# mitsuba-renderer/mitsuba2

Hardware: AMD Instinct MI355X
Metric: Msamples/sec (whole node), 1080p/512spp path integrator (higher is better)
Workload: dtype f32

## Files before the change

### mitsuba2_amd/csrc/device/resident_kernel.h

```cpp
#ifndef MIW_KERNEL
#define MIW_KERNEL __global__
#endif
MIW_KERNEL __launch_bounds__(MIW_BLOCK) void k_init_pixels(RenderParams P, U4 *st_out, uint32_t *pixel_out, InitArgs A) {
    uint32_t lane = blockIdx.x * blockDim.x + threadIdx.x;
    if (lane >= P.n_lanes) return;
    uint32_t tile = lane >> A.bs2_log2, i = lane & ((1u << A.bs2_log2) - 1u);
    uint32_t b = A.tile_list ? A.tile_list[tile] : tile;
    uint32_t bx = b % A.blocks_x, by = b / A.blocks_x;
    uint32_t x, y;
    morton_decode2(i, x, y);
    int32_t bw = P.film.crop_w - (int32_t) (bx * A.bs), bh = P.film.crop_h - (int32_t) (by * A.bs);
    if (bw > (int32_t) A.bs) bw = (int32_t) A.bs;
    if (bh > (int32_t) A.bs) bh = (int32_t) A.bs;
    if ((int32_t) x >= bw || (int32_t) y >= bh) {
        U4 st; st.x = st.y = 0; st.z = LF_DONE; st.w = 0;
        st_out[lane] = st; pixel_out[lane] = 0;
        return;
    }
    uint32_t px = (uint32_t) P.film.crop_x + bx * A.bs + x, py = (uint32_t) P.film.crop_y + by * A.bs + y;
    pixel_out[lane] = px | (py << 16);
    st_out[lane] = lane_seed_state(A.base_seed + (uint64_t) A.block_ids[b] * (uint64_t) (A.bs * A.bs) + i);
}

struct TileArgs {
    const uint32_t *tile_list; uint32_t blocks_x, bs, bs2_log2;
    uint32_t side;
    uint32_t geom16;
};

#ifndef MIW_PLACE_PIECES
#define MIW_PLACE_PIECES 4
#endif
template <bool Placed = true, bool Clock = false, bool Groups = false, bool Jobs = true>
struct QueueWork {
    const LaneQueues *Q; uint32_t *next_pixel; uint32_t n_lanes, spp, lane, warn_negative;
    const FilmRec *film; const float *thr;
    uint32_t nq, per, q, dry, t_fetch;
    __device__ __forceinline__ void init_queues(uint32_t queues) {
        nq = Placed ? queues : 1u; per = nq > 1u ? MIW_PLACE_PIECES * 64u : n_lanes; q = 0u; dry = 0; t_fetch = 0;
        ticks = 0; quarter = 0; tail_prio = 0; sample_end_ = spp;
        if (Jobs) job_pend() = 0u;
        if (Placed && Q->simd_ids) {
            const uint32_t hw = (uint32_t) __builtin_amdgcn_s_getreg(4 | (0 << 6) | (31 << 11)),
                           xcc = (uint32_t) __builtin_amdgcn_s_getreg(20 | (0 << 6) | (3 << 11));
            const uint32_t key = ((xcc & 15u) << 10) | (((hw >> 13) & 7u) << 7) | (((hw >> 12) & 1u) << 6) | (((hw >> 8) & 15u) << 2) | ((hw >> 4) & 3u);
            if (nq > 1u) { const uint32_t id = Q->simd_ids[1u + key]; q = id < nq ? id : key % nq; }
            else if ((threadIdx.x & 63u) == 0u) Q->simd_ids[1u + key] = 1u;
        }
    }
    uint32_t ticks, quarter, tail_prio, sample_end_; uint32_t *prog;
    __device__ __forceinline__ void tick(uint32_t sample_idx, bool has_pixel) {
        if (!tail_prio) { ++ticks; return; }
        if ((uint32_t) __builtin_amdgcn_readfirstlane((int) ++ticks) & 15u) return;
        if (has_pixel) atomicMin(prog, sample_idx);
        const uint32_t v = *prog;
        *prog = 0xffffffffu;
        const uint32_t v4 = 4u * v, se = sample_end_;
        uint32_t qtr = v == 0xffffffffu ? 3u : (v4 >= se ? 1u : 0u) + (v4 >= 2u * se ? 1u : 0u) + (v4 >= 3u * se ? 1u : 0u);
        qtr = (uint32_t) __builtin_amdgcn_readfirstlane((int) qtr);
        if (qtr == quarter) return;
        quarter = qtr;
        if (qtr == 0u) __builtin_amdgcn_s_setprio(3); else if (qtr == 1u) __builtin_amdgcn_s_setprio(2);
        else if (qtr == 2u) __builtin_amdgcn_s_setprio(1); else __builtin_amdgcn_s_setprio(0);
    }
    __device__ __forceinline__ void enable_tail_prio(uint32_t sample_end, uint32_t *wave_word) {
        tail_prio = 1u; sample_end_ = sample_end; quarter = 0; prog = wave_word; *prog = 0xffffffffu; __builtin_amdgcn_s_setprio(3);
    }
    typedef uint32_t U4v __attribute__((ext_vector_type(4)));
    __device__ __forceinline__ static uint32_t &job_pend() { __shared__ uint32_t s_job_pend[MIW_BLOCK]; return s_job_pend[threadIdx.x & (MIW_BLOCK - 1)]; }
    __device__ __forceinline__ bool exhausted() const { return !Jobs || !Q->job_chunk || job_pend() == 0xffffffffu; }
    __device__ __forceinline__ uint32_t job_end(uint32_t sample_idx, uint32_t sample_end) const {
        const uint32_t r = spp - sample_idx;
        return Jobs && (r & (r - 1u)) == 0u && r >= Q->job_min ? sample_idx : sample_end;
    }
    __device__ __forceinline__ bool fetch_job(uint32_t &pixel, U4 &st) {
        for (;;) {
            const uint32_t parked = job_pend();
            if (parked == 0xffffffffu) return false;
            uint32_t id = parked - 1u;
            const bool fresh = parked == 0u;
            const unsigned long long b = __ballot(fresh);
            if (fresh) {
                const uint32_t me = threadIdx.x & 63u, leader = (uint32_t) __ffsll((long long) b) - 1u;
                uint32_t base = 0;
                if (me == leader) base = atomicAdd(next_pixel, (uint32_t) __popcll(b));
                base = (uint32_t) __shfl((int) base, (int) leader, 64);
                id = base + __builtin_amdgcn_mbcnt_hi((uint32_t) (b >> 32), __builtin_amdgcn_mbcnt_lo((uint32_t) b, 0u));
                if (id >= Q->job_total) { job_pend() = 0xffffffffu; return false; }
            }
            const uint32_t j = id / n_lanes, slot = id - j * n_lanes;
            const uint32_t px = Q->pixel[slot];
            U4v w;
#if defined(__HIP_DEVICE_COMPILE__)
            asm volatile("global_load_dwordx4 %0, %1, off sc1\n\ts_waitcnt vmcnt(0)" : "=&v"(w) : "v"(Q->st + slot) : "memory");
#endif
            if (w.z & LF_DONE) { job_pend() = 0u; continue; }
            if (w.w != (j ? spp - (Q->job_pow >> (j - 1u)) : 0u)) { job_pend() = id + 1u; return false; }
            job_pend() = 0u;
            lane = slot; pixel = px;
            st.x = w.x; st.y = w.y; st.z = w.z; st.w = w.w;
            return true;
        }
    }
    __device__ __forceinline__ bool fetch(uint32_t &pixel, U4 &st) {
        if (Jobs && Q->job_chunk) return fetch_job(pixel, st);
        for (;;) {
            if (!Placed) {
                const unsigned long long b = __ballot(1);
                const uint32_t me = threadIdx.x & 63u, leader = (uint32_t) __ffsll((long long) b) - 1u;
                uint32_t base = 0;
                if (me == leader) base = atomicAdd(next_pixel, (uint32_t) __popcll(b));
                base = (uint32_t) __shfl((int) base, (int) leader, 64);
                const uint32_t l = base + __builtin_amdgcn_mbcnt_hi((uint32_t) (b >> 32), __builtin_amdgcn_mbcnt_lo((uint32_t) b, 0u));
                if (l >= n_lanes) return false;
                lane = l;
                st = Q->st[lane];
                if (st.z & LF_DONE) continue;
                pixel = Q->pixel[lane];
                return true;
            }
            if (dry >= nq) {
                if (nq > 1u) Q->simd_ids[0] = 1u;
                return false;
            }
            if (nq > 1u && __hip_atomic_load(Q->simd_ids, __ATOMIC_RELAXED, __HIP_MEMORY_SCOPE_AGENT)) { dry = nq; return false; }
            const unsigned long long all = __ballot(1);
            const uint32_t me = threadIdx.x & 63u, leader = (uint32_t) __ffsll((long long) all) - 1u;
            const uint32_t q_lead = (uint32_t) __shfl((int) q, (int) leader, 64);
// ... 3 lines not shown
            uint32_t base = 0;
            if (me == leader) base = atomicAdd(next_pixel + q, (uint32_t) __popcll(b));
            base = (uint32_t) __shfl((int) base, (int) leader, 64);
            const uint32_t idx = base + __builtin_amdgcn_mbcnt_hi((uint32_t) (b >> 32), __builtin_amdgcn_mbcnt_lo((uint32_t) b, 0u));
            uint32_t l = idx;
            if (nq > 1u) {
                const uint32_t piece = idx < per ? Q->piece_list[q * MIW_PLACE_PIECES + (idx >> 6)] : 0xffffffffu;
                if (piece == 0xffffffffu) { q = q + 1u == nq ? 0u : q + 1u; ++dry; continue; }
                l = Q->lane_sorted[piece * Q->piece_a + (idx & 63u) * Q->piece_b];
                if (l >= n_lanes) continue;
            } else if (l >= n_lanes) { ++dry; continue; }
            lane = l;
            st = Q->st[lane];
            if (st.z & LF_DONE) continue;
            pixel = Q->pixel[lane];
            if (Placed) t_fetch = cost_clock();
            return true;
        }
    }
    __device__ __forceinline__ uint32_t cost_clock() const {
        return Clock ? (uint32_t) (__builtin_amdgcn_s_memtime() >> 8) : ticks;
    }
    __device__ __forceinline__ void store(U4 st) {
        if (Jobs && Q->job_chunk) {
            unsigned long long *words = reinterpret_cast<unsigned long long *>(Q->st + lane);
            __hip_atomic_store(words, (unsigned long long) st.x | ((unsigned long long) st.y << 32), __ATOMIC_RELAXED, __HIP_MEMORY_SCOPE_AGENT);
            asm volatile("s_waitcnt vmcnt(0)" ::: "memory");
            __hip_atomic_store(words + 1, (unsigned long long) st.z | ((unsigned long long) st.w << 32), __ATOMIC_RELAXED, __HIP_MEMORY_SCOPE_AGENT);
            return;
        }
        Q->st[lane] = st;
        if (Placed && Q->lane_cost) Q->lane_cost[lane] = cost_clock() - t_fetch + 1u;
        if (Groups && Q->group_done && (st.z & LF_DONE)) {
            __threadfence();
            const uint32_t g = lane >> Q->group_shift;
            if (atomicAdd(Q->group_done + g, 1u) + 1u == Q->group_expected[g]) {
                __threadfence_system();
                __hip_atomic_store(Q->group_flag + g, 1u, __ATOMIC_RELEASE, __HIP_MEMORY_SCOPE_SYSTEM);
            }
        }
    }
    __device__ __forceinline__ void put(uint32_t pixel, uint32_t sample_idx, V2 pos, const float *aovs) {
        if (Q->log_rec) {
            LogSink16<const float *> sink{ Q->log_rec, thr, film, lane, spp, Q->log_rej & 255u, Q->log_rej >> 8 };
            sink(pixel, sample_idx, pos, aovs);
        } else {
            LogSink sink; sink.log_pos = Q->log_pos; sink.log_val = Q->log_val; sink.lane = lane; sink.spp = spp; sink.warn_negative = warn_negative;
            sink(0u, sample_idx, pos, aovs);
        }
    }
};

#ifndef MIW_DIRECT_WAVES
#define MIW_DIRECT_WAVES 3
#endif
#ifndef MIW_PACKET_WAVES_ALL
#define MIW_PACKET_WAVES_ALL 4
#endif
#ifndef MIW_PACKET_WAVES
#define MIW_PACKET_WAVES 5
#endif
template <bool UseLog, int Tiny, int Mats = MATS_ALL, bool Analytic = (Tiny == 0), uint32_t Integ = INTEG_PATH, bool Groups = false, int Waves = 0, uint32_t Feat = FEAT_ALL>
__global__ __launch_bounds__(MIW_BLOCK, Waves ? Waves : Integ == INTEG_DIRECT ? MIW_DIRECT_WAVES : Tiny ? ((Mats == MATS_DIFFUSE && !MIW_SPECTRAL) ? (Tiny == 2 ? MIW_PACKET_WAVES : 4) : MIW_PACKET_WAVES_ALL) : MIW_TREE_WAVES) void k_path_resident(RenderParams P, SceneView sc, LaneQueues Q, double *accum, Counters *cnt,
                                                               TraceLds cfg, uint32_t sample_end, TileArgs T, uint32_t *next_pixel) {
    extern __shared__ uint4 smem[];
    stage_to_lds(sc, cfg, smem);
    const float *thr = stage_thresholds(smem, cfg, UseLog && Q.log_rec ? Q.log_thr : nullptr);
    constexpr bool Frames = MIW_LDS_TABLES && UseLog && Tiny != 0 && Integ != INTEG_DIRECT;
#if MIW_LDS_TABLES
    if constexpr (UseLog && Tiny != 0) stage_tables<true, mats_lights(Mats), mats_full(Mats), Frames>(sc, cfg, smem);
#endif
#if defined(MIW_SECTION_PROFILE) && defined(__HIP_DEVICE_COMPILE__)
    if ((threadIdx.x & 63u) == 0) { unsigned long long *b_ = miw_sec_buf(); for (int i = 0; i < 15; ++i) b_[i] = 0; b_[15] = __builtin_amdgcn_s_memtime(); }
#endif
    const uint32_t lane = blockIdx.x * blockDim.x + threadIdx.x;
    double *tile = reinterpret_cast<double *>(smem + T.geom16);
    int tile_x0 = 0, tile_y0 = 0;
    if (!UseLog && T.side) {
        const uint32_t lane0 = blockIdx.x * blockDim.x, t = lane0 >> T.bs2_log2, q0 = lane0 & ((1u << T.bs2_log2) - 1u);
        const uint32_t b = T.tile_list ? T.tile_list[t] : t;
        uint32_t qx, qy;
        morton_decode2(q0, qx, qy);
        const int margin = (int) (T.side - 16u) / 2;
        tile_x0 = (int) ((b % T.blocks_x) * T.bs + qx) - margin;
        tile_y0 = (int) ((b / T.blocks_x) * T.bs + qy) - margin;
        for (uint32_t i = threadIdx.x; i < T.side * T.side * MIW_FILM_CHANNELS; i += blockDim.x) tile[i] = 0.0;
        __syncthreads();
    }
    LaneCounters local; local.segments = local.samples = local.shadow_rays = 0;
    auto tr2 = [&](V3 o, float mint, V3 dE, float maxtE, bool hasE, V3 dS, float maxtS, bool hasS, F4 &hE, bool &occS) {
        trace2<Tiny, Analytic, Integ != INTEG_DIRECT>(sc, cfg, smem, o, mint, dE, maxtE, hasE, dS, maxtS, hasS, hE, occS);
    };
    if (UseLog) {
        QueueWork<Tiny != 0, false, Groups> work; work.Q = &Q; work.next_pixel = next_pixel; work.n_lanes = P.n_lanes; work.spp = P.spp; work.lane = 0; work.warn_negative = P.film.warn_negative;
        work.film = &P.film; work.thr = thr; work.init_queues(cfg.queues ? cfg.queues : 1u);
        __shared__ uint32_t s_prog[MIW_BLOCK / 64];
        if (cfg.tail_prio) work.enable_tail_prio(sample_end, &s_prog[threadIdx.x >> 6]);
        if constexpr (Integ == INTEG_DIRECT) pixel_stream_render_direct<Mats, Analytic>(P, sc, sample_end, work, tr2, &local);
        else pixel_stream_render<Mats, Analytic, Frames, Feat>(P, sc, sample_end, work, tr2, &local);
    } else if (lane < P.n_lanes) {
        U4 st = Q.st[lane];
        if (!(st.z & LF_DONE)) {
            const uint32_t pixel = Q.pixel[lane];
            if (T.side) {
                TileAdd add; add.tile = tile; add.x0 = tile_x0; add.y0 = tile_y0; add.side = (int) T.side;
                SplatXYSink<TileAdd> sink; sink.film = &P.film; sink.add = add;
                st = pixel_render<Integ, mats_nested(Mats) ? Mats : MATS_ALL>(P, sc, pixel, st, sample_end, tr2, sink, &local);
            } else {
                FilmAdd add; add.accum = accum;
                SplatSink<FilmAdd> sink; sink.film = &P.film; sink.add = add;
                st = pixel_render<Integ, mats_nested(Mats) ? Mats : MATS_ALL>(P, sc, pixel, st, sample_end, tr2, sink, &local);
            }
            Q.st[lane] = st;
        }
    }
    if (!UseLog && T.side) {
        __syncthreads();
        const int n = (int) (T.side * T.side);
        for (int i = (int) threadIdx.x; i < n * MIW_FILM_CHANNELS; i += (int) blockDim.x) {
            const double v = tile[i];
            if (v == 0.0) continue;
            const int texel = i / MIW_FILM_CHANNELS, k = i - texel * MIW_FILM_CHANNELS;
// ... 16 lines not shown
```

### mitsuba2_amd/csrc/device/trace.h

```cpp

struct TraceLds {
    uint32_t nodes_staged;
    uint32_t tris_staged;
    uint32_t brute;
    uint32_t leaves;
    uint32_t stack;
    uint32_t stack16;
    uint32_t shade_num, shade_den;
    uint32_t node_exit, tri_exit;
    uint32_t queues;
    uint32_t tail_prio;
    uint32_t thr16;
    uint32_t tab16;
    uint32_t tab_words[12];
    uint32_t env_top_count, env_top_base, env_top_words;
    uint32_t pool_claim_min;
    uint32_t pool16, stat16;
    uint32_t light_words;
};

struct alignas(16) LeafBox { float p[6]; uint32_t mask_lo, mask_hi; };
static_assert(sizeof(LeafBox) == 32, "LeafBox must be 32 bytes");

struct alignas(16) TriPacket { float p0[3], e1[3], e2[3]; uint32_t prim; uint32_t pad[2]; };
// ... 357 lines not shown
        return bvh_intersect<AnyHit>(node_at, tri_at, r, h, prim_ctx(sc));
    } else {
#if MIW_LDS_TOP
        uint32_t ns = cfg.nodes_staged;
        auto node_at = [lnodes, gnodes, ns](int32_t i) -> const BvhNode & {
            return (uint32_t) i < ns ? lnodes[i] : gnodes[i];
        };
#else
        auto node_at = [gnodes](int32_t i) -> const BvhNode & { return gnodes[i]; };
#endif
        auto tri_at = [gtris](uint32_t i) -> const Tri & { return gtris[i]; };
        if (cfg.stack) {
            int32_t *stack = reinterpret_cast<int32_t *>(const_cast<uint4 *>(smem) + cfg.stack16) + threadIdx.x;
#if MIW_WALK == 0
            return bvh_intersect_stack<AnyHit, Analytic>(node_at, tri_at, stack, o, d, mint, maxt, h, prim_ctx(sc));
#else
            return bvh_intersect_ww<AnyHit, Analytic, MIW_WALK == 2>(node_at, tri_at, stack, o, d, mint, maxt, h, prim_ctx(sc));
#endif
        }
        return bvh_intersect<AnyHit>(node_at, tri_at, r, h, prim_ctx(sc));
    }
}

template <int Tiny, bool Analytic = true, bool LeafPairs = false>
__device__ __forceinline__ void trace2(const SceneView &sc, TraceLds cfg, const uint4 *smem,
                                       V3 o, float mint, V3 dE, float maxtE, bool hasE,
                                       V3 dS, float maxtS, bool hasS, F4 &hit_out, bool &occ_out) {
    Hit h; h.t = MIW_INFINITY; h.u = h.v = 0.f; h.tri = MIW_MISS; h.prim = 0xffffffffu;
    bool occ = false;
    if (Tiny && cfg.leaves) {
        using Mask = typename std::conditional<Tiny == 2, uint32_t, unsigned long long>::type;
        auto lowest = [](Mask m) -> uint32_t {
            return Tiny == 2 ? (uint32_t) __ffs((int) (uint32_t) m) - 1u : (uint32_t) __ffsll((long long) m) - 1u;
        };
        const TriPacket *pk = reinterpret_cast<const TriPacket *>(smem);
        const LeafBox *lb = reinterpret_cast<const LeafBox *>(smem + sc.tri_count * (sizeof(TriPacket) / 16));
        const TriBounds *tb = packet_bounds(sc, cfg, smem);
        const FastRay rE = fast_ray(o, dE, mint), rS = fast_ray(o, dS, mint);
        const float wideE = widen(maxtE), wideS = widen(maxtS);
        Mask mE = 0, mS = 0;
#if MIW_OCTANT_BOXES
        const LeafBox *lbE = lb + ray_octant(rE), *lbS = lb + ray_octant(rS);
        using LeafOperands = typename std::conditional<LeafPairs, LeafRay, FastRay>::type;
        LeafOperands qE, qS;
        if constexpr (LeafPairs) { qE = leaf_ray(rE, o); qS = leaf_ray(rS, o); } else { qE = rE; qS = rS; }
        for (uint32_t i = 0; i < cfg.leaves; ++i) {
            const LeafBox &bE = lbE[8u * i], &bS = lbS[8u * i];
            const Mask bits = Tiny == 2 ? (Mask) bE.mask_lo : (Mask) (bE.mask_lo | ((unsigned long long) bE.mask_hi << 32));
            if (leaf_box_test_octant(bE, qE, wideE)) mE |= bits;
            if (leaf_box_test_octant(bS, qS, wideS)) mS |= bits;
        }
#else
        for (uint32_t i = 0; i < cfg.leaves; ++i) {
// ... 68 lines not shown
```

### mitsuba2_amd/csrc/kernel_pick.h

```cpp
#pragma once

namespace miw_pick {

enum : int { ALL = 0, DIFFUSE = 1, PLAIN = 2, TRIO = 3, NESTED = 4, LIGHTS = 5 };

struct Facts {
    bool tiny;
    bool small;
    bool diffuse_only, trio, nested, textured, lights_on;
    bool no_rects;
    bool trio_on;
};

struct Pick {
    int tiny;
    int mats;
    bool analytic;
};
inline bool operator==(const Pick &a, const Pick &b) { return a.tiny == b.tiny && a.mats == b.mats && a.analytic == b.analytic; }

inline bool trio_kernel(const Facts &f) { return f.trio && f.trio_on && f.no_rects && !f.textured; }

inline Pick resident_path(const Facts &f, bool with_trio) {
    if (f.tiny && f.diffuse_only) return { f.small ? 2 : 1, DIFFUSE, false };
// ... 3 lines not shown
    if (f.tiny) return { f.small ? 2 : 1, PLAIN, false };
    if (with_trio && trio_kernel(f)) return { 0, TRIO, false };
    return { 0, PLAIN, !f.no_rects };
}

inline Pick resident_direct(const Facts &f) {
    const int mats = f.lights_on ? LIGHTS : f.nested ? NESTED : f.textured ? ALL : PLAIN;
    return { f.tiny ? 1 : 0, mats, !f.tiny };
}

inline Pick resident_atomic(const Facts &f) {
    return { f.tiny ? 1 : 0, f.lights_on ? LIGHTS : f.nested ? NESTED : ALL, !f.tiny };
}

inline Pick tree_class(const Facts &f) {
    if (f.lights_on) return { 0, LIGHTS, true };
    if (f.nested) return { 0, NESTED, true };
    if (f.textured) return { 0, ALL, true };
    if (trio_kernel(f)) return { 0, TRIO, false };
    return { 0, PLAIN, !f.no_rects };
}

enum : unsigned { FEAT_ENV = 1u, FEAT_SHAPE_NORMALS = 2u, FEAT_EMITTER_NORMALS = 4u, FEAT_MOMENT = 8u, FEAT_ALL = 15u, FEAT_NONE = 0u };

inline unsigned packet_features(bool has_env, bool shape_normals, bool emitter_normals, bool moment) {
    return (has_env ? FEAT_ENV : 0u) | (shape_normals ? FEAT_SHAPE_NORMALS : 0u) | (emitter_normals ? FEAT_EMITTER_NORMALS : 0u) | (moment ? FEAT_MOMENT : 0u);
}
inline bool packet_features_exist(unsigned mask) { return mask == FEAT_ALL || mask == FEAT_NONE; }
inline unsigned packet_features_kernel(unsigned needed, bool lean_on) { return lean_on && packet_features_exist(needed) ? needed : (unsigned) FEAT_ALL; }
inline bool packet_lean_class(const Pick &p) { return p.tiny != 0 && !p.analytic && (p.mats == DIFFUSE || p.mats == PLAIN); }

}
```

### mitsuba2_amd/csrc/miw/scene.h

```cpp
#pragma once
#include "base.h"
#include "shape.h"
#include "bsdf.h"
#include "envmap.h"
#include "light.h"
#include "../kernel_pick.h"

namespace miw {

#define MIW_MISS 0xffffffffu

struct BvhNode {
    float lo0[3], hi0[3];
    float lo1[3], hi1[3];
    int32_t child0, child1;
    int32_t parent;
    int32_t pad;
};

struct ShapeRec {
    uint32_t bsdf;
    int32_t  emitter;
    uint32_t flags;
    uint32_t pad;
};

struct EmitterRec {
    TexRec radiance;
    uint32_t shape;
    uint32_t tri_first;
    uint32_t tri_count;
    uint32_t valid_lo, valid_hi;
    float sum, normalization;
    uint32_t flags;
    uint32_t type;
};
enum : uint32_t { SHAPE_HAS_NORMALS = 1u, SHAPE_HAS_TEXCOORDS = 8u };
enum : uint32_t { FEAT_ENV = miw_pick::FEAT_ENV, FEAT_SHAPE_NORMALS = miw_pick::FEAT_SHAPE_NORMALS, FEAT_EMITTER_NORMALS = miw_pick::FEAT_EMITTER_NORMALS,
                  FEAT_MOMENT = miw_pick::FEAT_MOMENT, FEAT_ALL = miw_pick::FEAT_ALL, FEAT_NONE = miw_pick::FEAT_NONE };

struct SceneView {
    const BvhNode *nodes;   uint32_t node_count;
    const Tri     *tris;    uint32_t tri_count;
    const float   *tri_vn;
    const float   *tri_uv;
    const ShapeRec *shapes; uint32_t shape_count;
    const BsdfRec  *bsdfs;  uint32_t bsdf_count;
    const EmitterRec *emitters; uint32_t emitter_count;
    float emitter_count_f, emitter_count_inv;
    const float *emit_tri;
    const float *emit_vnorm;
    const float *emit_pmf, *emit_cdf;
    const EnvmapRec *env;
    const AnalyticRec *rects;   uint32_t rect_count;
    const BitmapRec *bitmaps;
    const float *bsdf_tables;
    float accept_pad;
    const void *tri_bounds;
    const void *leaf_boxes;
    const struct Bvh4Node *nodes4;
    const struct Bvh8Node *nodes8;
    const float *env_top; uint32_t env_top_count, env_top_base;
// ... 278 lines not shown
```

### mitsuba2_amd/csrc/miwave.hip

```cpp
#include <hip/hip_runtime.h>
#include <stdio.h>
#include <stdlib.h>
#include <string.h>
#include <stdarg.h>
#include <string>
#include <vector>
#include <chrono>
#include <atomic>
#include <cmath>
#include <map>
#include <string>
#include <algorithm>

#include "../../include/miwave.h"
#include "kernel_pick.h"
#if defined(MIW_CLASS_PART) || defined(MIW_AOV_UNIT)
#define MIW_KERNELS_ONLY 1
#endif
#if defined(MIW_SECTION_PROFILE)
__device__ unsigned long long g_sections[16];
#endif
#if defined(MIW_PHASE_STATS)
__device__ unsigned long long g_phase_stats[15];
#endif
// ... 107 lines not shown
struct KnobInfo { const char *name, *what; };
static const KnobInfo g_knobs[] = {
    { "MIW_DEBUG", "1: diagnostics on stderr (LDS layout, builder statistics, phase statistics of -DMIW_PHASE_STATS builds)" },
    { "MIW_DEBUG_ALLOC", "1: mi_bvh_build times its uploads and allocations" },
    { "MIW_DEVICE_BUILDER", "mi_bvh_build quality 0: sah (default) | lbvh: which device builder runs" },
    { "MIW_SAH_HUGE", "0: the device SAH sweep bins every candidate in one workgroup (round 4's form)" },
    { "MIW_LBVH_LEAF", "radix tree: triangles per leaf" },
    { "MIW_MAX_LEAF", "host SAH builder: triangles per leaf" },
    { "MIW_NO_STACK", "1: no LDS-stack walk (stackless BVH2 walk, wavefront plan)" },
    { "MIW_BVH4", "0: no 4-wide tree (the phase machine steps through the BVH2)" },
    { "MIW_BVH4_FAN", "2 | 3 | 4: widest node the 4-wide collapse may build" },
    { "MIW_BVH4_HOST", "1: the 4-wide tree is collapsed on the host from the read-back BVH2" },
    { "MIW_BVH8", "0: mi_bvh_build skips the 8-wide tree / mi_render keeps the 4-wide walk" },
    { "MIW_STACK8_FULL", "1: the 8-wide walk keeps the 16-entry LDS column instead of one entry per tree level" },
    { "MIW_ENV_TOP", "0: the environment warp's top levels are not staged in LDS" },
    { "MIW_PHASED", "0: tree scenes take the lock-step kernel instead of the phase machine" },
    { "MIW_PHASED_WAVES", "3 | 4: wavefronts per SIMD the phase machine is launched for" },
    { "MIW_TRIO", "0: MATS_PLAIN kernels where the MATS_TRIO class would do" },
    { "MIW_SHADE_VOTE", "num:den of the phase machine's shade vote" },
    { "MIW_LOOP_EXIT", "node:triangle hand-over ratios of the phase machine's walk loops" },
    { "MIW_POOLED", "1: tree scenes take k_path_pooled (walk jobs pooled across the workgroup; experimental, slower: DESIGN.md)" },
    { "MIW_POOL_SHAPE", "12x1 | 8x2: wavefronts per workgroup x pixels per lane of k_path_pooled" },
    { "MIW_POOL_VOTE", "shade_min:walk_min:node_min:tri_min:claim_min of k_path_pooled" },
    { "MIW_TAIL_PRIO", "0: no least-progress-first wave priorities" },
    { "MIW_WG_PER_CU", "workgroups per CU of the packet kernels' persistent grid" },
    { "MIW_PLACE", "0: shards of about one pixel per lane skip the measuring launch + placed queues" },
    { "MIW_JOB_CHUNK", "smallest chunk of a full frame's pixel jobs, in samples (a power of two; default 64, the phase machine 32): the pixels' sample streams are cut into halving chunks drawn chunk-major from one queue; 0: a job = all the samples of a pixel" },
    { "MIW_JOB_CHUNK_FORCE", "1: chunk jobs whatever the frame's size (tests of the hand-over between lanes)" },
    { "MIW_LEAN", "0: a packet scene without environment map and vertex normals, rendered without the moment integrator, keeps the full path kernel instead of its lean twin (kernel_pick.h: packet_features)" },
    { "MIW_PACKET_SHARD4", "0: a plain-diffuse packet job of at most four wavefronts of pixels per SIMD keeps the five-wavefront (96-register) kernel" },
    { "MIW_PLACE_MEASURE", "divisor: the measuring launch runs spp / divisor samples" },
    { "MIW_PLACE_SPREAD", "0 | 1: placed pieces = consecutive sorted lanes | one lane of every cost stratum" },
    { "MIW_STREAM", "0: plan 1 walks with one kernel per list slice instead of the persistent stream kernel" },
    { "MIW_FILM_LEGACY", "1: the 24-byte position log + k_film_blocks for every filter" },
    { "MIW_FILM_LANES", "0 | 1 | 2: k_film_lanes off / over the tile-interleaved log / over [lane][sample]" },
    { "MIW_FILM_QUADS", "0 | 24 | 28 | 42 | 44: k_film_quads group shape (0: off)" },
    { "MIW_FILM_COLUMNS", "0 | 42 | 44 | 82: k_film_columns group shape" },
    { "MIW_FILM_GROUP", "2 | 3 | 4: k_film_groups group shape" },
    { "MIW_FL_NT", "0: k_film_lanes reads the log with plain instead of streaming loads" },
    { "MIW_FILM_OVERLAP", "1: part of the film replay of a full Cornell-class frame is queued on three more streams beside the path kernel, sets of 64-tile groups each behind the flags their last pixels raise (default 0: measured +0 - 1 %); 2: without the waits (timing probe: the film is the previous frame's)" },
    { "MIW_FILM_OVERLAP_SET", "groups of 64 tiles per launch of that replay (default 4)" },
    { "MIW_FILM_OVERLAP_ROOM", "workgroups the path kernel's grid is short of filling the device while the replay runs beside it (default 32: one per CU on 32 CUs)" },
    { "MIW_FILM_OVERLAP_LEAN", "0: the launches of that replay are the 168-register kernel (default 1: the 128-register form)" },
    { "MIW_FILM_OVERLAP_BESIDE", "groups of 64 tiles replayed beside the path kernel; the rest in one launch after it (default: three quarters)" },
    { "MIW_FILM_OVERLAP_PRIO", "s_setprio of the replay wavefronts that run beside the path kernel, 0 .. 3 (default 0)" },
    { "MIW_FQ_U", "2 | 4 | 8: records per trip of k_film_quads" },
    { "MIW_RCCL", "0: mi_film_reduce never uses RCCL (device add)" },
    { "MIW_RCCL_FORCE", "1: mi_film_reduce takes the RCCL branch for one context too (tests)" }
};
struct Options {
    std::map<std::string, std::string> v;
    void from_env() { for (const KnobInfo &k : g_knobs) if (const char *e = getenv(k.name)) v[k.name] = e; }
// ... 1764 lines not shown
        }
        TileArgs TA; memset(&TA, 0, sizeof TA);
        size_t tile_bytes = 0;
        if (film_mode == 2 && bs >= 16) {
            TA.tile_list = A.tile_list; TA.blocks_x = blocks_x; TA.bs = bs; TA.bs2_log2 = bs2_log2;
            TA.side = 16u + 2u * std::max<uint32_t>((uint32_t) cfg->filter_border, (uint32_t) floorf(cfg->filter_radius + .5f));
            TA.geom16 = (uint32_t) ((c->lds_bytes + 15) / 16);
            tile_bytes = (size_t) TA.geom16 * 16 - c->lds_bytes + (size_t) TA.side * TA.side * MIW_FILM_CHANNELS * sizeof(double);
            if (c->lds_bytes + tile_bytes > 64 * 1024) {
#define MIW_ATOMIC_ATTR(T, M, A, I) HIP_TRY(c, hipFuncSetAttribute((const void *) k_path_resident<false, T, M, A, I>, hipFuncAttributeMaxDynamicSharedMemorySize, (int) (c->lds_bytes + tile_bytes)));
                MIW_ATOMIC_LIST(MIW_ATOMIC_ATTR)
#undef MIW_ATOMIC_ATTR
            }
        }
        const uint32_t sync_every = 8;
        uint32_t launches = 0;
        bool place_stats_due = false;
        const int overlap_mode = ropt.num("MIW_FILM_OVERLAP", 0);
        const bool overlap = overlap_mode != 0 && c->overlap_state != 0 && film_mode == 1 && FP.rec16 && FP.film_lanes != 0 && FP.log_il != 0 && !place && !phased  && tiny && c->diffuse_only && !MIW_SPECTRAL && !direct  &&
                             per_launch >= cfg->spp && cfg->timeout_s <= 0.f && n_tiles > 0;
        for (uint32_t done = 0; done < cfg->spp; ) {
            uint32_t end = cfg->spp - done < per_launch ? cfg->spp : done + per_launch;
            uint32_t feat_launched = FEAT_ALL;
            if (film_mode == 1) {
                HIP_TRY(c, hipMemsetAsync(c->d_next_pixel.p, 0, c->d_next_pixel.n * sizeof(uint32_t), s));
                rcfg.queues = 1u; Q.lane_cost = nullptr; Q.lane_sorted = nullptr; Q.piece_list = nullptr; Q.simd_ids = nullptr;
                if (overlap && done == 0) {
                    mi_status os = film_replay_setup(c, cfg, s, FP, n_tiles, bs, bs2_log2, blocks_x, blocks_y, replay);
                    if (os == MI_OK) os = overlap_prepare(c, cfg, s, n_tiles, bs, blocks_x, Q, bs2_log2);
                    if (os != MI_OK) return os;
                    if (Q.group_done) HIP_TRY(c, hipEventRecord(c->ev_fork, s));
                }
                Q.job_chunk = Q.job_pow = Q.job_total = 0u; Q.job_min = 0x80000000u;
                if ((tiny || (phased && MIW_PHASED_JOBS != 0)) && !pooled_fits && !place && !overlap && done == 0 && per_launch >= cfg->spp && cfg->timeout_s <= 0.f) {
                    uint32_t jmin = tiny ? 64u : 32u;
                    if (const char *e = ropt.get("MIW_JOB_CHUNK")) { const uint32_t v = (uint32_t) std::max(0, atoi(e)); jmin = (v & (v - 1u)) ? 0u : v; }
                    bool enough = (uint64_t) n_lanes * 5u >= (uint64_t) 6u * 64u * res_waves * n_simd;
                    if (ropt.on("MIW_JOB_CHUNK_FORCE")) enough = true;
                    uint32_t pow2 = 1u;
                    while (pow2 * 2u < cfg->spp) pow2 *= 2u;
                    uint64_t chunks = 1u;
                    for (uint32_t r = pow2; jmin && r >= jmin && r < cfg->spp; r >>= 1) ++chunks;
                    if (jmin && enough && chunks >= 2u && (uint64_t) n_lanes * chunks < (1ull << 31)) {
                        Q.job_chunk = jmin; Q.job_min = jmin; Q.job_pow = pow2; Q.job_total = (uint32_t) ((uint64_t) n_lanes * chunks);
                        K.job_chunk = jmin; K.job_chunks = (uint32_t) chunks;
                    }
// ... 16 lines not shown
                    if (nqueues) {
                    std::vector<uint32_t> &list = c->h_piece_list;
                    list.assign((size_t) nqueues * MIW_PLACE_PIECES, 0xffffffffu);
                    for (uint32_t i = 0; i < n_pieces; ++i) {
                        const uint32_t round = i / nqueues, k = i % nqueues, qd = (round & 1u) ? nqueues - 1u - k : k;
                        list[(size_t) qd * MIW_PLACE_PIECES + round] = i;
                    }
                    HIP_TRY(c, c->d_piece_list.resize(list.size()));
                    HIP_TRY(c, hipMemcpyAsync(c->d_piece_list.p, list.data(), list.size() * sizeof(uint32_t), hipMemcpyHostToDevice, s));
                    HIP_TRY(c, hipMemcpyAsync(c->d_simd_ids.p, ids.data(), ids.size() * sizeof(uint32_t), hipMemcpyHostToDevice, s));
                    rcfg.queues = nqueues; Q.piece_list = c->d_piece_list.p; Q.lane_sorted = c->d_lane_sorted.p; Q.simd_ids = c->d_simd_ids.p;
                    K.placed = 1u;
                    }
                }
                unsigned wg_per_cu = std::max(4u, direct ? 4u : (unsigned) res_waves);
                if (const char *e = ropt.get("MIW_WG_PER_CU")) wg_per_cu = (unsigned) std::max(1, atoi(e));
                unsigned room = 0u;
                if (Q.group_done) { room = 32u; if (const char *e = ropt.get("MIW_FILM_OVERLAP_ROOM")) room = (unsigned) std::max(0, atoi(e)); }
                const unsigned resident = (unsigned) c->cu_count * (direct ? (unsigned) MIW_DIRECT_WAVES : (unsigned) res_waves);
                const unsigned full = room ? std::min((unsigned) c->cu_count * wg_per_cu, resident) : (unsigned) c->cu_count * wg_per_cu;
                const dim3 pgrid(std::min<unsigned>(grid.x, full > 2u * room ? full - room : full));
                K.path_kernel = phased ? (c->view.nodes4 ? 1u : 3u) : 0u;
                const dim3 phgrid(std::min<unsigned>(grid.x, (unsigned) c->cu_count * (unsigned) ph_waves));
                rcfg.tail_prio = 1u;
                if (ropt.off("MIW_TAIL_PRIO")) rcfg.tail_prio = 0u;
                TraceLds ph_cfg = rcfg;
                ph_cfg.shade_num = 2; ph_cfg.shade_den = c->have_env ? 4 : 3;
                if (const char *e = ropt.get("MIW_SHADE_VOTE")) { int a = 0, b = 0; if (sscanf(e, "%d:%d", &a, &b) == 2 && a > 0 && b > 0) { ph_cfg.shade_num = (uint32_t) a; ph_cfg.shade_den = (uint32_t) b; } }
                ph_cfg.node_exit = c->have_env ? 2u : 1u; ph_cfg.tri_exit = c->have_env ? 3u : 2u;
                if (const char *e = ropt.get("MIW_LOOP_EXIT")) { int a = 0, b = 0; if (sscanf(e, "%d:%d", &a, &b) == 2 && a >= 0 && b >= 0) { ph_cfg.node_exit = (uint32_t) a; ph_cfg.tri_exit = (uint32_t) b; } }
#define MIW_PHASED_LAUNCH_(M, A, WV, W, PL) MIW_TIMED(6, hipLaunchKernelGGL((k_path_phased<M, A, MIW_PHASE_SPEC != 0, WV, W, PL>), phgrid, block, rlds, s, P, (W) == 2 ? view8 : c->view, Q, c->d_cnt.p, ph_cfg, end, c->d_next_pixel.p))
#define MIW_PHASED_LAUNCH(M, A, W) do { if (ph_waves == 4) MIW_PHASED_LAUNCH_(M, A, 4, W, false); else MIW_PHASED_LAUNCH_(M, A, 3, W, false); } while (0)
                K.tree_width = phased ? (phased8 ? 8u : (c->view.nodes4 ? 4u : 2u)) : 0u;
#if MIW_SPECTRAL
                const bool pooled = false;
                if (pooled) { }
#else
                const bool pooled = phased8 && !place && pooled_fits;
                if (pooled) {
                    TraceLds pcfg = layp.cfg; pcfg.queues = 1u; pcfg.tail_prio = ph_cfg.tail_prio;
                    pcfg.shade_num = 48; pcfg.shade_den = 16; pcfg.node_exit = 40u; pcfg.tri_exit = 20u; pcfg.pool_claim_min = 8u;
                    if (const char *e = ropt.get("MIW_POOL_VOTE")) { int a = 0, b = 0, n = 0, t = 0, m = 0; if (sscanf(e, "%d:%d:%d:%d:%d", &a, &b, &n, &t, &m) == 5 && a > 0 && b >= 0) { pcfg.shade_num = (uint32_t) a; pcfg.shade_den = (uint32_t) b; pcfg.node_exit = (uint32_t) n; pcfg.tri_exit = (uint32_t) t; pcfg.pool_claim_min = (uint32_t) std::max(m, 1); } }
                    const unsigned NL = (unsigned) pool_nw * 64u;
                    const dim3 qgrid(std::min<unsigned>((n_lanes + NL - 1u) / NL, (unsigned) c->cu_count)), qblock(NL);
                    SceneView pview = view8;
                    if (c->lights_on) return fail(c, MI_ERR_INVALID, "render: the pooled kernel (MI_PATH_KERNEL_POOLED) does not serve scenes with point / spot / directional / constant emitters");
                    if (c->nested) return fail(c, MI_ERR_INVALID, "render: the pooled kernel (MI_PATH_KERNEL_POOLED) does not serve scenes with mask / blendbsdf / null / thindielectric records");
                    const miw_pick::Pick pick = miw_pick::tree_class(facts);
// ... 8 lines not shown
                else
                if (phased && !c->view.nodes4) MIW_PHASED_LAUNCH(MATS_TRIO, false, 0);
                else if (phased) {
                    const miw_pick::Pick pick = miw_pick::tree_class(facts);
                    const int wide = phased8 ? 2 : 1;
#define MIW_PHASED_PICKED(M, A, WV, W, PL) if (pick.mats == (M) && pick.analytic == (A) && ph_waves == (WV) && wide == (W) && place == (PL)) MIW_PHASED_LAUNCH_(M, A, WV, W, PL); else
                    MIW_PHASED_LIST(MIW_PHASED_PICKED) return fail(c, MI_ERR_STATE, "render: no k_path_phased<%d, %d, ., %d, %d, %d> in the library", pick.mats, (int) pick.analytic, ph_waves, wide, (int) place);
#undef MIW_PHASED_PICKED
                }
#undef MIW_PHASED_LAUNCH
#undef MIW_PHASED_LAUNCH_
                else if (Q.group_done && c->view.tri_count <= 32u)
                    MIW_TIMED(6, hipLaunchKernelGGL((k_path_resident<true, 2, MATS_DIFFUSE, false, INTEG_PATH, true>), pgrid, block, rlds, s, P, c->view, Q, (double *) nullptr, c->d_cnt.p, rcfg, end, TA, c->d_next_pixel.p));
                else if (Q.group_done)
                    MIW_TIMED(6, hipLaunchKernelGGL((k_path_resident<true, 1, MATS_DIFFUSE, false, INTEG_PATH, true>), pgrid, block, rlds, s, P, c->view, Q, (double *) nullptr, c->d_cnt.p, rcfg, end, TA, c->d_next_pixel.p));
                else if (packet_shard4 && !Q.group_done && feat == FEAT_NONE) {
                    feat_launched = FEAT_NONE;
                    MIW_TIMED(6, hipLaunchKernelGGL((k_path_resident<true, 2, MATS_DIFFUSE, false, INTEG_PATH, false, 4, FEAT_NONE>), pgrid, block, rlds, s, P, c->view, Q, (double *) nullptr, c->d_cnt.p, rcfg, end, TA, c->d_next_pixel.p));
                }
                else if (packet_shard4 && !Q.group_done)
                    MIW_TIMED(6, hipLaunchKernelGGL((k_path_resident<true, 2, MATS_DIFFUSE, false, INTEG_PATH, false, 4>), pgrid, block, rlds, s, P, c->view, Q, (double *) nullptr, c->d_cnt.p, rcfg, end, TA, c->d_next_pixel.p));
                else {
                    const miw_pick::Pick pick = direct ? miw_pick::resident_direct(facts) : miw_pick::resident_path(facts, false);
#define MIW_LEAN_LAUNCH(T, M) if (feat == FEAT_NONE && !direct && MIW_PICKED(T, M, false)) { feat_launched = FEAT_NONE; MIW_TIMED(6, hipLaunchKernelGGL((k_path_resident<true, T, M, false, INTEG_PATH, false, 0, FEAT_NONE>), pgrid, block, rlds, s, P, c->view, Q, (double *) nullptr, c->d_cnt.p, rcfg, end, TA, c->d_next_pixel.p)); } else
                    MIW_LEAN_LIST(MIW_LEAN_LAUNCH)
#undef MIW_LEAN_LAUNCH
#define MIW_RESIDENT_LAUNCH(T, M, A, I) if (integ == (I) && MIW_PICKED(T, M, A)) MIW_TIMED(6, hipLaunchKernelGGL((k_path_resident<true, T, M, A, I>), pgrid, block, (T) != 0 ? rlds : rlds_plain, s, P, c->view, Q, (double *) nullptr, c->d_cnt.p, rcfg, end, TA, c->d_next_pixel.p)); else
                    MIW_RESIDENT_LIST(MIW_RESIDENT_LAUNCH) return fail(c, MI_ERR_STATE, "render: no k_path_resident<true, %d, %d, %d, %u> in the library", pick.tiny, pick.mats, (int) pick.analytic, integ);
#undef MIW_RESIDENT_LAUNCH
                }
            } else {
                const miw_pick::Pick pick = miw_pick::resident_atomic(facts);
#define MIW_ATOMIC_LAUNCH(T, M, A, I) if (integ == (I) && MIW_PICKED(T, M, A)) MIW_TIMED(6, hipLaunchKernelGGL((k_path_resident<false, T, M, A, I>), grid, block, c->lds_bytes + tile_bytes, s, P, c->view, Q, c->d_accum.p, c->d_cnt.p, c->lds_cfg, end, TA, (uint32_t *) nullptr)); else
                MIW_ATOMIC_LIST(MIW_ATOMIC_LAUNCH) return fail(c, MI_ERR_STATE, "render: no k_path_resident<false, %d, %d, %d, %u> in the library", pick.tiny, pick.mats, (int) pick.analytic, integ);
#undef MIW_ATOMIC_LAUNCH
            }
            if (Q.group_done) {
                const mi_status os = overlap_enqueue(c, ropt, P, s, T, replay, n_tiles, overlap_mode != 2);
                if (os != MI_OK) return os;
                if (c->replay_enqueued) { K.film_overlapped = 1u; K.film_groups = c->replay_launches; }
                Q.group_done = nullptr; Q.group_expected = nullptr; Q.group_flag = nullptr;
            }
            if (ropt.get("MIW_DEBUG") && tiny && !phased) fprintf(stderr, "[miwave] packet path kernel launched: scene features 0x%x of 0x%x compiled in (mask chosen for the render: 0x%x)\n", feat_launched, (uint32_t) FEAT_ALL, feat);
            K.n_path++; K.iterations++;
            done = end;
            if ((++launches % sync_every == 0 || cfg->timeout_s > 0.f || c->cancel.load()) && done < cfg->spp) {
                HIP_TRY(c, hipGetLastError());
                HIP_TRY(c, hipStreamSynchronize(s));
                T.drain();
                if (c->cancel.load() || out_of_time()) { result = MI_ERR_CANCELLED; break; }
            }
        }
        HIP_TRY(c, hipGetLastError());
        Counters sum;
        mi_status rs = read_counters(sum);
        if (rs != MI_OK) return rs;
        if (place_stats_due) {
            std::vector<uint32_t> all(n_lanes); uint32_t first_lane = 0, px = 0;
            HIP_TRY(c, hipMemcpyAsync(all.data(), c->d_cost_sorted.p, (size_t) n_lanes * sizeof(uint32_t), hipMemcpyDeviceToHost, s));
            HIP_TRY(c, hipMemcpyAsync(&first_lane, c->d_lane_sorted.p, sizeof(uint32_t), hipMemcpyDeviceToHost, s));
            HIP_TRY(c, hipStreamSynchronize(s));
            if (first_lane < n_lanes) HIP_TRY(c, hipMemcpy(&px, c->q_pixel.p + first_lane, sizeof(uint32_t), hipMemcpyDeviceToHost));
            double csum = 0.0; uint32_t with = 0;
            for (uint32_t v : all) if (v) { csum += (double) v; ++with; }
            K.place_cost_max = all.empty() ? 0u : all[0]; K.place_cost_mean = with ? csum / with : 0.0; K.place_max_pixel = px;
            K.place_cost_unit = phased ? 1u : 0u; K.place_measure_spp = measure_end;
// ... 153 lines not shown
```

Baseline: 4924.

## Add frame-twin packet kernel with launch facts compiled in; drop tail priorities for chunk jobs

Adds a specialised instantiation of the resident packet path kernel that hard-codes the conditions of a full-frame chunk-job launch: one job queue, 16-byte log records, no tail priorities, leaf filtering on, no group counts. Runtime branches and the tail-priority bookkeeping drop out, which may lower register pressure and instruction count. It also turns tail priorities off by default for packet launches that use chunk jobs. The cost is another kernel instantiation (larger binary and compile time) and extra selection logic on the host.

```diff
diff --git a/mitsuba2_amd/csrc/device/resident_kernel.h b/mitsuba2_amd/csrc/device/resident_kernel.h
--- a/mitsuba2_amd/csrc/device/resident_kernel.h
+++ b/mitsuba2_amd/csrc/device/resident_kernel.h
@@ -31,8 +31,9 @@
 #ifndef MIW_PLACE_PIECES
 #define MIW_PLACE_PIECES 4
 #endif
-template <bool Placed = true, bool Clock = false, bool Groups = false, bool Jobs = true>
+template <bool Placed = true, bool Clock = false, bool Groups = false, bool Jobs = true, bool Frame = false>
 struct QueueWork {
+    static_assert(!Frame || (!Placed && !Groups && Jobs), "the frame twin: one queue of chunk jobs, no group counts");
     const LaneQueues *Q; uint32_t *next_pixel; uint32_t n_lanes, spp, lane, warn_negative;
     const FilmRec *film; const float *thr;
     uint32_t nq, per, q, dry, t_fetch;
@@ -50,6 +51,7 @@
     }
     uint32_t ticks, quarter, tail_prio, sample_end_; uint32_t *prog;
     __device__ __forceinline__ void tick(uint32_t sample_idx, bool has_pixel) {
+        if (Frame) return;
         if (!tail_prio) { ++ticks; return; }
         if ((uint32_t) __builtin_amdgcn_readfirstlane((int) ++ticks) & 15u) return;
         if (has_pixel) atomicMin(prog, sample_idx);
@@ -68,7 +70,7 @@
     }
     typedef uint32_t U4v __attribute__((ext_vector_type(4)));
     __device__ __forceinline__ static uint32_t &job_pend() { __shared__ uint32_t s_job_pend[MIW_BLOCK]; return s_job_pend[threadIdx.x & (MIW_BLOCK - 1)]; }
-    __device__ __forceinline__ bool exhausted() const { return !Jobs || !Q->job_chunk || job_pend() == 0xffffffffu; }
+    __device__ __forceinline__ bool exhausted() const { return (!Frame && (!Jobs || !Q->job_chunk)) || job_pend() == 0xffffffffu; }
     __device__ __forceinline__ uint32_t job_end(uint32_t sample_idx, uint32_t sample_end) const {
         const uint32_t r = spp - sample_idx;
         return Jobs && (r & (r - 1u)) == 0u && r >= Q->job_min ? sample_idx : sample_end;
@@ -103,7 +105,7 @@
         }
     }
     __device__ __forceinline__ bool fetch(uint32_t &pixel, U4 &st) {
-        if (Jobs && Q->job_chunk) return fetch_job(pixel, st);
+        if (Frame || (Jobs && Q->job_chunk)) return fetch_job(pixel, st);
         for (;;) {
             if (!Placed) {
                 const unsigned long long b = __ballot(1);
@@ -153,7 +155,7 @@
         return Clock ? (uint32_t) (__builtin_amdgcn_s_memtime() >> 8) : ticks;
     }
     __device__ __forceinline__ void store(U4 st) {
-        if (Jobs && Q->job_chunk) {
+        if (Frame || (Jobs && Q->job_chunk)) {
             unsigned long long *words = reinterpret_cast<unsigned long long *>(Q->st + lane);
             __hip_atomic_store(words, (unsigned long long) st.x | ((unsigned long long) st.y << 32), __ATOMIC_RELAXED, __HIP_MEMORY_SCOPE_AGENT);
             asm volatile("s_waitcnt vmcnt(0)" ::: "memory");
@@ -172,7 +174,7 @@
         }
     }
     __device__ __forceinline__ void put(uint32_t pixel, uint32_t sample_idx, V2 pos, const float *aovs) {
-        if (Q->log_rec) {
+        if (Frame || Q->log_rec) {
             LogSink16<const float *> sink{ Q->log_rec, thr, film, lane, spp, Q->log_rej & 255u, Q->log_rej >> 8 };
             sink(pixel, sample_idx, pos, aovs);
         } else {
@@ -194,9 +196,11 @@
 template <bool UseLog, int Tiny, int Mats = MATS_ALL, bool Analytic = (Tiny == 0), uint32_t Integ = INTEG_PATH, bool Groups = false, int Waves = 0, uint32_t Feat = FEAT_ALL>
 __global__ __launch_bounds__(MIW_BLOCK, Waves ? Waves : Integ == INTEG_DIRECT ? MIW_DIRECT_WAVES : Tiny ? ((Mats == MATS_DIFFUSE && !MIW_SPECTRAL) ? (Tiny == 2 ? MIW_PACKET_WAVES : 4) : MIW_PACKET_WAVES_ALL) : MIW_TREE_WAVES) void k_path_resident(RenderParams P, SceneView sc, LaneQueues Q, double *accum, Counters *cnt,
                                                                TraceLds cfg, uint32_t sample_end, TileArgs T, uint32_t *next_pixel) {
+    constexpr bool Frame = (Feat & FEAT_FRAME) != 0;
+    static_assert(!Frame || (UseLog && Tiny != 0 && !Analytic && Integ == INTEG_PATH && !Groups && Waves == 0 && Feat == FEAT_FRAME), "a frame twin is the twin of a lean packet kernel");
     extern __shared__ uint4 smem[];
     stage_to_lds(sc, cfg, smem);
-    const float *thr = stage_thresholds(smem, cfg, UseLog && Q.log_rec ? Q.log_thr : nullptr);
+    const float *thr = stage_thresholds(smem, cfg, UseLog && (Frame || Q.log_rec) ? Q.log_thr : nullptr);
     constexpr bool Frames = MIW_LDS_TABLES && UseLog && Tiny != 0 && Integ != INTEG_DIRECT;
 #if MIW_LDS_TABLES
     if constexpr (UseLog && Tiny != 0) stage_tables<true, mats_lights(Mats), mats_full(Mats), Frames>(sc, cfg, smem);
@@ -220,15 +224,17 @@
     }
     LaneCounters local; local.segments = local.samples = local.shadow_rays = 0;
     auto tr2 = [&](V3 o, float mint, V3 dE, float maxtE, bool hasE, V3 dS, float maxtS, bool hasS, F4 &hE, bool &occS) {
-        trace2<Tiny, Analytic, Integ != INTEG_DIRECT>(sc, cfg, smem, o, mint, dE, maxtE, hasE, dS, maxtS, hasS, hE, occS);
+        trace2<Tiny, Analytic, Integ != INTEG_DIRECT, Frame>(sc, cfg, smem, o, mint, dE, maxtE, hasE, dS, maxtS, hasS, hE, occS);
     };
     if (UseLog) {
-        QueueWork<Tiny != 0, false, Groups> work; work.Q = &Q; work.next_pixel = next_pixel; work.n_lanes = P.n_lanes; work.spp = P.spp; work.lane = 0; work.warn_negative = P.film.warn_negative;
+        QueueWork<Tiny != 0 && !Frame, false, Groups, true, Frame> work; work.Q = &Q; work.next_pixel = next_pixel; work.n_lanes = P.n_lanes; work.spp = P.spp; work.lane = 0; work.warn_negative = P.film.warn_negative;
         work.film = &P.film; work.thr = thr; work.init_queues(cfg.queues ? cfg.queues : 1u);
-        __shared__ uint32_t s_prog[MIW_BLOCK / 64];
-        if (cfg.tail_prio) work.enable_tail_prio(sample_end, &s_prog[threadIdx.x >> 6]);
+        if constexpr (!Frame) {
+            __shared__ uint32_t s_prog[MIW_BLOCK / 64];
+            if (cfg.tail_prio) work.enable_tail_prio(sample_end, &s_prog[threadIdx.x >> 6]);
+        }
         if constexpr (Integ == INTEG_DIRECT) pixel_stream_render_direct<Mats, Analytic>(P, sc, sample_end, work, tr2, &local);
-        else pixel_stream_render<Mats, Analytic, Frames, Feat>(P, sc, sample_end, work, tr2, &local);
+        else pixel_stream_render<Mats, Analytic, Frames, Feat & FEAT_ALL>(P, sc, sample_end, work, tr2, &local);
     } else if (lane < P.n_lanes) {
         U4 st = Q.st[lane];
         if (!(st.z & LF_DONE)) {
diff --git a/mitsuba2_amd/csrc/device/trace.h b/mitsuba2_amd/csrc/device/trace.h
--- a/mitsuba2_amd/csrc/device/trace.h
+++ b/mitsuba2_amd/csrc/device/trace.h
@@ -403,13 +403,13 @@
     }
 }
 
-template <int Tiny, bool Analytic = true, bool LeafPairs = false>
+template <int Tiny, bool Analytic = true, bool LeafPairs = false, bool Filtered = false>
 __device__ __forceinline__ void trace2(const SceneView &sc, TraceLds cfg, const uint4 *smem,
                                        V3 o, float mint, V3 dE, float maxtE, bool hasE,
                                        V3 dS, float maxtS, bool hasS, F4 &hit_out, bool &occ_out) {
     Hit h; h.t = MIW_INFINITY; h.u = h.v = 0.f; h.tri = MIW_MISS; h.prim = 0xffffffffu;
     bool occ = false;
-    if (Tiny && cfg.leaves) {
+    if (Tiny && (Filtered || cfg.leaves)) {
         using Mask = typename std::conditional<Tiny == 2, uint32_t, unsigned long long>::type;
         auto lowest = [](Mask m) -> uint32_t {
             return Tiny == 2 ? (uint32_t) __ffs((int) (uint32_t) m) - 1u : (uint32_t) __ffsll((long long) m) - 1u;
diff --git a/mitsuba2_amd/csrc/kernel_pick.h b/mitsuba2_amd/csrc/kernel_pick.h
--- a/mitsuba2_amd/csrc/kernel_pick.h
+++ b/mitsuba2_amd/csrc/kernel_pick.h
@@ -49,6 +49,7 @@
 }
 
 enum : unsigned { FEAT_ENV = 1u, FEAT_SHAPE_NORMALS = 2u, FEAT_EMITTER_NORMALS = 4u, FEAT_MOMENT = 8u, FEAT_ALL = 15u, FEAT_NONE = 0u };
+enum : unsigned { FEAT_FRAME = 16u };
 
 inline unsigned packet_features(bool has_env, bool shape_normals, bool emitter_normals, bool moment) {
     return (has_env ? FEAT_ENV : 0u) | (shape_normals ? FEAT_SHAPE_NORMALS : 0u) | (emitter_normals ? FEAT_EMITTER_NORMALS : 0u) | (moment ? FEAT_MOMENT : 0u);
@@ -57,4 +58,17 @@
 inline unsigned packet_features_kernel(unsigned needed, bool lean_on) { return lean_on && packet_features_exist(needed) ? needed : (unsigned) FEAT_ALL; }
 inline bool packet_lean_class(const Pick &p) { return p.tiny != 0 && !p.analytic && (p.mats == DIFFUSE || p.mats == PLAIN); }
 
+struct LaunchFacts {
+    bool job_chunks;
+    bool log_rec16;
+    bool one_queue;
+    bool tail_prio;
+    bool leaf_filter;
+    bool group_counts;
+};
+inline bool frame_twin(const Pick &p, bool direct, unsigned feat, const LaunchFacts &l, bool twin_on) {
+    return twin_on && !direct && feat == FEAT_NONE && packet_lean_class(p) &&
+           l.job_chunks && l.log_rec16 && l.one_queue && !l.tail_prio && l.leaf_filter && !l.group_counts;
 }
+
+}
diff --git a/mitsuba2_amd/csrc/miw/scene.h b/mitsuba2_amd/csrc/miw/scene.h
--- a/mitsuba2_amd/csrc/miw/scene.h
+++ b/mitsuba2_amd/csrc/miw/scene.h
@@ -37,7 +37,8 @@
 };
 enum : uint32_t { SHAPE_HAS_NORMALS = 1u, SHAPE_HAS_TEXCOORDS = 8u };
 enum : uint32_t { FEAT_ENV = miw_pick::FEAT_ENV, FEAT_SHAPE_NORMALS = miw_pick::FEAT_SHAPE_NORMALS, FEAT_EMITTER_NORMALS = miw_pick::FEAT_EMITTER_NORMALS,
-                  FEAT_MOMENT = miw_pick::FEAT_MOMENT, FEAT_ALL = miw_pick::FEAT_ALL, FEAT_NONE = miw_pick::FEAT_NONE };
+                  FEAT_MOMENT = miw_pick::FEAT_MOMENT, FEAT_ALL = miw_pick::FEAT_ALL, FEAT_NONE = miw_pick::FEAT_NONE,
+                  FEAT_FRAME = miw_pick::FEAT_FRAME };
 
 struct SceneView {
     const BvhNode *nodes;   uint32_t node_count;
diff --git a/mitsuba2_amd/csrc/miwave.hip b/mitsuba2_amd/csrc/miwave.hip
--- a/mitsuba2_amd/csrc/miwave.hip
+++ b/mitsuba2_amd/csrc/miwave.hip
@@ -153,12 +153,13 @@
     { "MIW_POOLED", "1: tree scenes take k_path_pooled (walk jobs pooled across the workgroup; experimental, slower: DESIGN.md)" },
     { "MIW_POOL_SHAPE", "12x1 | 8x2: wavefronts per workgroup x pixels per lane of k_path_pooled" },
     { "MIW_POOL_VOTE", "shade_min:walk_min:node_min:tri_min:claim_min of k_path_pooled" },
-    { "MIW_TAIL_PRIO", "0: no least-progress-first wave priorities" },
+    { "MIW_TAIL_PRIO", "0: no least-progress-first wave priorities; 1: also in a packet kernel's launch of chunk jobs, which runs without them by default (and then keeps its lean kernel instead of the frame twin)" },
     { "MIW_WG_PER_CU", "workgroups per CU of the packet kernels' persistent grid" },
     { "MIW_PLACE", "0: shards of about one pixel per lane skip the measuring launch + placed queues" },
     { "MIW_JOB_CHUNK", "smallest chunk of a full frame's pixel jobs, in samples (a power of two; default 64, the phase machine 32): the pixels' sample streams are cut into halving chunks drawn chunk-major from one queue; 0: a job = all the samples of a pixel" },
     { "MIW_JOB_CHUNK_FORCE", "1: chunk jobs whatever the frame's size (tests of the hand-over between lanes)" },
     { "MIW_LEAN", "0: a packet scene without environment map and vertex normals, rendered without the moment integrator, keeps the full path kernel instead of its lean twin (kernel_pick.h: packet_features)" },
+    { "MIW_FRAME_TWIN", "0: a full frame of chunk jobs keeps the lean twin of its packet path kernel instead of the frame twin, which has the facts of such a launch compiled in (kernel_pick.h: frame_twin)" },
     { "MIW_PACKET_SHARD4", "0: a plain-diffuse packet job of at most four wavefronts of pixels per SIMD keeps the five-wavefront (96-register) kernel" },
     { "MIW_PLACE_MEASURE", "divisor: the measuring launch runs spp / divisor samples" },
     { "MIW_PLACE_SPREAD", "0 | 1: placed pieces = consecutive sorted lanes | one lane of every cost stratum" },
@@ -1969,6 +1970,7 @@
         for (uint32_t done = 0; done < cfg->spp; ) {
             uint32_t end = cfg->spp - done < per_launch ? cfg->spp : done + per_launch;
             uint32_t feat_launched = FEAT_ALL;
+            bool frame_launched = false;
             if (film_mode == 1) {
                 HIP_TRY(c, hipMemsetAsync(c->d_next_pixel.p, 0, c->d_next_pixel.n * sizeof(uint32_t), s));
                 rcfg.queues = 1u; Q.lane_cost = nullptr; Q.lane_sorted = nullptr; Q.piece_list = nullptr; Q.simd_ids = nullptr;
@@ -2031,8 +2033,8 @@
                 const dim3 pgrid(std::min<unsigned>(grid.x, full > 2u * room ? full - room : full));
                 K.path_kernel = phased ? (c->view.nodes4 ? 1u : 3u) : 0u;
                 const dim3 phgrid(std::min<unsigned>(grid.x, (unsigned) c->cu_count * (unsigned) ph_waves));
-                rcfg.tail_prio = 1u;
-                if (ropt.off("MIW_TAIL_PRIO")) rcfg.tail_prio = 0u;
+                rcfg.tail_prio = tiny && Q.job_chunk ? 0u : 1u;
+                if (const char *e = ropt.get("MIW_TAIL_PRIO")) rcfg.tail_prio = atoi(e) != 0 ? 1u : 0u;
                 TraceLds ph_cfg = rcfg;
                 ph_cfg.shade_num = 2; ph_cfg.shade_den = c->have_env ? 4 : 3;
                 if (const char *e = ropt.get("MIW_SHADE_VOTE")) { int a = 0, b = 0; if (sscanf(e, "%d:%d", &a, &b) == 2 && a > 0 && b > 0) { ph_cfg.shade_num = (uint32_t) a; ph_cfg.shade_den = (uint32_t) b; } }
@@ -2087,6 +2089,13 @@
                     MIW_TIMED(6, hipLaunchKernelGGL((k_path_resident<true, 2, MATS_DIFFUSE, false, INTEG_PATH, false, 4>), pgrid, block, rlds, s, P, c->view, Q, (double *) nullptr, c->d_cnt.p, rcfg, end, TA, c->d_next_pixel.p));
                 else {
                     const miw_pick::Pick pick = direct ? miw_pick::resident_direct(facts) : miw_pick::resident_path(facts, false);
+                    miw_pick::LaunchFacts lf;
+                    lf.job_chunks = Q.job_chunk != 0u; lf.log_rec16 = Q.log_rec != nullptr; lf.one_queue = rcfg.queues == 1u; lf.tail_prio = rcfg.tail_prio != 0u;
+                    lf.leaf_filter = c->lds_cfg.leaves != 0u; lf.group_counts = Q.group_done != nullptr;
+                    const bool frame = miw_pick::frame_twin(pick, direct, feat, lf, !ropt.off("MIW_FRAME_TWIN"));
+#define MIW_FRAME_LAUNCH(T, M) if (frame && MIW_PICKED(T, M, false)) { feat_launched = FEAT_NONE; frame_launched = true; MIW_TIMED(6, hipLaunchKernelGGL((k_path_resident<true, T, M, false, INTEG_PATH, false, 0, FEAT_FRAME>), pgrid, block, rlds, s, P, c->view, Q, (double *) nullptr, c->d_cnt.p, rcfg, end, TA, c->d_next_pixel.p)); } else
+                    MIW_LEAN_LIST(MIW_FRAME_LAUNCH)
+#undef MIW_FRAME_LAUNCH
 #define MIW_LEAN_LAUNCH(T, M) if (feat == FEAT_NONE && !direct && MIW_PICKED(T, M, false)) { feat_launched = FEAT_NONE; MIW_TIMED(6, hipLaunchKernelGGL((k_path_resident<true, T, M, false, INTEG_PATH, false, 0, FEAT_NONE>), pgrid, block, rlds, s, P, c->view, Q, (double *) nullptr, c->d_cnt.p, rcfg, end, TA, c->d_next_pixel.p)); } else
                     MIW_LEAN_LIST(MIW_LEAN_LAUNCH)
 #undef MIW_LEAN_LAUNCH
@@ -2107,6 +2116,7 @@
                 Q.group_done = nullptr; Q.group_expected = nullptr; Q.group_flag = nullptr;
             }
             if (ropt.get("MIW_DEBUG") && tiny && !phased) fprintf(stderr, "[miwave] packet path kernel launched: scene features 0x%x of 0x%x compiled in (mask chosen for the render: 0x%x)\n", feat_launched, (uint32_t) FEAT_ALL, feat);
+            if (ropt.get("MIW_DEBUG") && tiny && !phased) fprintf(stderr, "[miwave] packet path kernel launched: frame twin %s\n", frame_launched ? "yes (chunk jobs, one queue, 16-byte log, no tail priorities, leaf filter compiled in)" : "no");
             K.n_path++; K.iterations++;
             done = end;
             if ((++launches % sync_every == 0 || cfg->timeout_s > 0.f || c->cancel.load()) && done < cfg->spp) {
```

Measured after the change: 5016, median of 6. 1.02x the previous value.
